# jluuser/PyTorch-VAE

Hardware: AMD Instinct MI355X
Metric: train images/sec @64x64x3 bs256 (curve tensors [B,64,6], SURVEY.md s0) (higher is better)
Workload: dtype f32; 1 GPU; C2: stage2_vq.yaml model with num_quantizers=1 K=512 D=64 N=64; full train step (fwd+loss+bwd+clip+AdamW+EMA), dropout 0.1, loss weights at epoch 100; per_gpu_batch=256, global_batch=256, seq_len=64, parallelism=dp1, hipgraph=True, params=43115078

## Files before the change

### pytorch-vae_amd/csrc/attention.hip

```cpp
#include "common.h"

namespace {

__device__ __forceinline__ int kmap(int r, int h) { return (r & 3) + 8 * (r >> 2) + 4 * h; }

__device__ __forceinline__ f32x4 ld4_guard(const float* p, bool ok) {
    f32x4 z = {0.f, 0.f, 0.f, 0.f};
    return ok ? *reinterpret_cast<const f32x4*>(p) : z;
}

struct AttnArgs {
    const float* Q; int ldq;
    const float* K; int ldk;
    const float* V; int ldv;
    float* O; int ldo;
    float* LSE;
    const unsigned char* kvalid;
    int B, nh, T, S;
    long long qbs, kbs, vbs;
    float scale;
    DropCfg drop;
    const float* dO; int lddo;
    float* Dsum;
    float* dQ; int lddq;
// ... 819 lines not shown
        hipError_t e = hipFuncSetAttribute(reinterpret_cast<const void*>(&attn_bwd_small4_kernel<DH>),
                                           hipFuncAttributeMaxDynamicSharedMemorySize, (int)smem);
        if (e != hipSuccess) {
            vqh_set_error(hipGetErrorString(e));
            return VQH_ERR_LAUNCH;
        }
        attr_set = true;
    }
    hipLaunchKernelGGL((attn_bwd_small4_kernel<DH>), dim3(1, a.nh, a.B), dim3(256), smem, stream, a);
    VQH_LAUNCH_CHECK();
    return VQH_OK;
}

template <int DH>
int launch_bwd_small(const AttnArgs& a, hipStream_t stream) {
    if (!(g_attn_flags & 2)) return launch_bwd_small4<DH>(a, stream);
    static bool attr_set = false;
    const size_t smem = (size_t)(4 * 64 * (DH + 4) + 3 * 64) * sizeof(float);
    if (!attr_set) {
        hipError_t e = hipFuncSetAttribute(reinterpret_cast<const void*>(&attn_bwd_small_kernel<DH>),
                                           hipFuncAttributeMaxDynamicSharedMemorySize, (int)smem);
        if (e != hipSuccess) {
            vqh_set_error(hipGetErrorString(e));
            return VQH_ERR_LAUNCH;
        }
        attr_set = true;
    }
    hipLaunchKernelGGL((attn_bwd_small_kernel<DH>), dim3(1, a.nh, a.B), dim3(256), smem, stream, a);
    VQH_LAUNCH_CHECK();
    return VQH_OK;
}

int g_attn_flags = 0;

}

extern "C" int vqh_attn_set_flags(int flags) { const int old = g_attn_flags; g_attn_flags = flags; return old; }

extern "C" int vqh_attn_fwd(const float* Q, int ldq, const float* K, int ldk, const float* V, int ldv, float* O,
                            int ldo, float* LSE, const unsigned char* kvalid, int B, int nh, int T, int S, int dh,
                            int qkv_shared, const unsigned long long* rng_state, unsigned drop_site, float drop_p,
                            hipStream_t stream) {
    VQH_CHECK_ARG(B >= 0 && nh > 0 && T >= 0 && S >= 0, "vqh_attn_fwd: bad shape");
    VQH_CHECK_ARG(dh == 16 || dh == 32 || dh == 64, "vqh_attn_fwd: head dim must be 16/32/64");
    if (B == 0 || T == 0) return VQH_OK;
    VQH_CHECK_ARG(S > 0, "vqh_attn_fwd: no keys");
    VQH_CHECK_ARG(Q && K && V && O, "vqh_attn_fwd: null pointer");
    VQH_CHECK_ARG(aligned16(Q, ldq) && aligned16(K, ldk) && aligned16(V, ldv), "vqh_attn_fwd: operands must be 16-byte aligned");
    VQH_CHECK_ARG(drop_p == 0.f || rng_state, "vqh_attn_fwd: dropout needs rng_state");
    AttnArgs a{};
    a.Q = Q; a.ldq = ldq; a.K = K; a.ldk = ldk; a.V = V; a.ldv = ldv; a.O = O; a.ldo = ldo; a.LSE = LSE;
    a.kvalid = kvalid; a.B = B; a.nh = nh; a.T = T; a.S = S; a.scale = 1.0f / sqrtf((float)dh);
    a.qbs = (qkv_shared & 1) ? 0 : (long long)T * ldq; a.kbs = (qkv_shared & 2) ? 0 : (long long)S * ldk; a.vbs = (qkv_shared & 2) ? 0 : (long long)S * ldv;
    a.drop = make_drop(rng_state, drop_site, drop_p);
    if (T <= 64 && S <= 64 && aligned16(O, ldo) && !(g_attn_flags & 1)) {
        dim3 grid(1, nh, B);
        if (dh == 64 && !(g_attn_flags & (2 | 4))) {
            static bool attr_set = false;
            const int smem = 2 * ax::IMG + 2 * 128 * 4;
            if (!attr_set) {
                hipError_t e = hipFuncSetAttribute(reinterpret_cast<const void*>(&attn_fwd_small_x3_kernel),
                                                   hipFuncAttributeMaxDynamicSharedMemorySize, smem);
                if (e != hipSuccess) { vqh_set_error(hipGetErrorString(e)); return VQH_ERR_LAUNCH; }
                attr_set = true;
            }
            hipLaunchKernelGGL(attn_fwd_small_x3_kernel, grid, dim3(256), smem, stream, a);
            VQH_LAUNCH_CHECK();
            return VQH_OK;
        }
        if (!(g_attn_flags & 2)) {
            switch (dh) {
                case 16: hipLaunchKernelGGL((attn_fwd_small4_kernel<16>), grid, dim3(256), 0, stream, a); break;
                case 32: hipLaunchKernelGGL((attn_fwd_small4_kernel<32>), grid, dim3(256), 0, stream, a); break;
                default: hipLaunchKernelGGL((attn_fwd_small4_kernel<64>), grid, dim3(256), 0, stream, a); break;
            }
            VQH_LAUNCH_CHECK();
            return VQH_OK;
        }
        switch (dh) {
            case 16: hipLaunchKernelGGL((attn_fwd_small_kernel<16>), grid, dim3(128), 0, stream, a); break;
            case 32: hipLaunchKernelGGL((attn_fwd_small_kernel<32>), grid, dim3(128), 0, stream, a); break;
            default: hipLaunchKernelGGL((attn_fwd_small_kernel<64>), grid, dim3(128), 0, stream, a); break;
        }
        VQH_LAUNCH_CHECK();
        return VQH_OK;
    }
    const int NWq = (T >= 128) ? 4 : 2;
    dim3 grid((T + 32 * NWq - 1) / (32 * NWq), nh, B);
    if (dh == 64 && !(g_attn_flags & 4) && aligned16(O, ldo)) {
        static bool attr_x3[2] = {false, false};
        const void* fn = (NWq == 4) ? reinterpret_cast<const void*>(&attn_fwd_x3_kernel<4>) : reinterpret_cast<const void*>(&attn_fwd_x3_kernel<2>);
        if (!attr_x3[NWq == 4]) {
            hipError_t e = hipFuncSetAttribute(fn, hipFuncAttributeMaxDynamicSharedMemorySize, 2 * ax::IMG);
            if (e != hipSuccess) { vqh_set_error(hipGetErrorString(e)); return VQH_ERR_LAUNCH; }
            attr_x3[NWq == 4] = true;
        }
        if (NWq == 4) hipLaunchKernelGGL((attn_fwd_x3_kernel<4>), grid, dim3(256), 2 * ax::IMG, stream, a);
// ... 15 lines not shown
}

extern "C" int vqh_attn_bwd(const float* Q, int ldq, const float* K, int ldk, const float* V, int ldv,
                            const float* O, int ldo, const float* LSE, const float* dO, int lddo, float* Dsum,
                            float* dQ, int lddq, float* dK, int lddk, float* dV, int lddv,
                            const unsigned char* kvalid, int B, int nh, int T, int S, int dh, int qkv_shared,
                            const unsigned long long* rng_state, unsigned drop_site, float drop_p,
                            hipStream_t stream) {
    VQH_CHECK_ARG(B >= 0 && nh > 0 && T >= 0 && S >= 0, "vqh_attn_bwd: bad shape");
    VQH_CHECK_ARG(dh == 16 || dh == 32 || dh == 64, "vqh_attn_bwd: head dim must be 16/32/64");
    if (B == 0 || T == 0 || S == 0) return VQH_OK;
    VQH_CHECK_ARG(Q && K && V && O && LSE && dO && Dsum && dQ && dK && dV, "vqh_attn_bwd: null pointer");
    VQH_CHECK_ARG(aligned16(Q, ldq) && aligned16(K, ldk) && aligned16(V, ldv) && aligned16(O, ldo) && aligned16(dO, lddo),
                  "vqh_attn_bwd: operands must be 16-byte aligned");
    VQH_CHECK_ARG(drop_p == 0.f || rng_state, "vqh_attn_bwd: dropout needs rng_state");
    AttnArgs a{};
    a.Q = Q; a.ldq = ldq; a.K = K; a.ldk = ldk; a.V = V; a.ldv = ldv; a.O = const_cast<float*>(O); a.ldo = ldo;
    a.LSE = const_cast<float*>(LSE); a.kvalid = kvalid; a.B = B; a.nh = nh; a.T = T; a.S = S;
    a.scale = 1.0f / sqrtf((float)dh);
    a.qbs = (qkv_shared & 1) ? 0 : (long long)T * ldq; a.kbs = (qkv_shared & 2) ? 0 : (long long)S * ldk; a.vbs = (qkv_shared & 2) ? 0 : (long long)S * ldv;
    a.drop = make_drop(rng_state, drop_site, drop_p);
    a.dO = dO; a.lddo = lddo; a.Dsum = Dsum; a.dQ = dQ; a.lddq = lddq; a.dK = dK; a.lddk = lddk; a.dV = dV; a.lddv = lddv;
    if (T <= 64 && S <= 64 && aligned16(dQ, lddq) && aligned16(dK, lddk) && aligned16(dV, lddv) && !(g_attn_flags & 1)) {
        int rc = VQH_OK;
        if (dh == 64 && !(g_attn_flags & (2 | 4))) {
            static bool attr_set = false;
            const int smem = 2 * 64 * (ax::DH + 4) * 4 + 64 * (ax::DH + 4) * 4;
            if (!attr_set) {
                hipError_t e = hipFuncSetAttribute(reinterpret_cast<const void*>(&attn_bwd_small_x3_kernel),
                                                   hipFuncAttributeMaxDynamicSharedMemorySize, smem);
                if (e != hipSuccess) { vqh_set_error(hipGetErrorString(e)); return VQH_ERR_LAUNCH; }
                attr_set = true;
            }
            hipLaunchKernelGGL(attn_bwd_small_x3_kernel, dim3(1, nh, B), dim3(256), smem, stream, a);
            VQH_LAUNCH_CHECK();
            return VQH_OK;
        }
        switch (dh) {
            case 16: rc = launch_bwd_small<16>(a, stream); break;
            case 32: rc = launch_bwd_small<32>(a, stream); break;
            default: rc = launch_bwd_small<64>(a, stream); break;
        }
        return rc;
    }
    const int NWq = (T >= 128) ? 4 : 2, NWk = (S >= 128) ? 4 : 2;
    dim3 gq((T + 32 * NWq - 1) / (32 * NWq), nh, B), gk((S + 32 * NWk - 1) / (32 * NWk), nh, B);
    if (dh == 64 && !(g_attn_flags & 4) && aligned16(dQ, lddq) && aligned16(dK, lddk) && aligned16(dV, lddv)) {
        static bool attr_b[4] = {false, false, false, false};
        const int smem_q = 2 * ax::IMG, smem_k = 2 * ax::IMG + 3 * 64 * 4;
        const void* fq = (NWq == 4) ? reinterpret_cast<const void*>(&attn_bwd_dq_x3_kernel<4>) : reinterpret_cast<const void*>(&attn_bwd_dq_x3_kernel<2>);
        const void* fk = (NWk == 4) ? reinterpret_cast<const void*>(&attn_bwd_dkv_x3_kernel<4>) : reinterpret_cast<const void*>(&attn_bwd_dkv_x3_kernel<2>);
        if (!attr_b[NWq == 4]) {
            hipError_t e = hipFuncSetAttribute(fq, hipFuncAttributeMaxDynamicSharedMemorySize, smem_q);
            if (e != hipSuccess) { vqh_set_error(hipGetErrorString(e)); return VQH_ERR_LAUNCH; }
            attr_b[NWq == 4] = true;
        }
        if (!attr_b[2 + (NWk == 4)]) {
            hipError_t e = hipFuncSetAttribute(fk, hipFuncAttributeMaxDynamicSharedMemorySize, smem_k);
            if (e != hipSuccess) { vqh_set_error(hipGetErrorString(e)); return VQH_ERR_LAUNCH; }
            attr_b[2 + (NWk == 4)] = true;
        }
        if (NWq == 4) hipLaunchKernelGGL((attn_bwd_dq_x3_kernel<4>), gq, dim3(256), smem_q, stream, a);
        else hipLaunchKernelGGL((attn_bwd_dq_x3_kernel<2>), gq, dim3(128), smem_q, stream, a);
        if (NWk == 4) hipLaunchKernelGGL((attn_bwd_dkv_x3_kernel<4>), gk, dim3(256), smem_k, stream, a);
        else hipLaunchKernelGGL((attn_bwd_dkv_x3_kernel<2>), gk, dim3(128), smem_k, stream, a);
        VQH_LAUNCH_CHECK();
// ... 19 lines not shown
```

### pytorch-vae_amd/csrc/attention_x3.inc

```
typedef unsigned ax_u32x2 __attribute__((ext_vector_type(2)));
typedef unsigned ax_u32x4 __attribute__((ext_vector_type(4)));
typedef short ax_s16x4 __attribute__((ext_vector_type(4)));
typedef __bf16 ax_bf16x8 __attribute__((ext_vector_type(8)));
typedef __bf16 ax_bf16x2 __attribute__((ext_vector_type(2)));
typedef float ax_f32x2 __attribute__((ext_vector_type(2)));

__device__ __forceinline__ void ax_split2(float a0, float a1, unsigned& h, unsigned& m, unsigned& l) {
    h = __builtin_bit_cast(unsigned, __builtin_convertvector(ax_f32x2{a0, a1}, ax_bf16x2));
    const float r0 = a0 - __uint_as_float(h << 16), r1 = a1 - __uint_as_float(h & 0xffff0000u);
    m = __builtin_bit_cast(unsigned, __builtin_convertvector(ax_f32x2{r0, r1}, ax_bf16x2));
    const float s0 = r0 - __uint_as_float(m << 16), s1 = r1 - __uint_as_float(m & 0xffff0000u);
    l = __builtin_bit_cast(unsigned, __builtin_convertvector(ax_f32x2{s0, s1}, ax_bf16x2));
}

namespace ax {
constexpr int DH = 64, CK = 64;
constexpr int PLANE = CK * DH * 2;
constexpr int IMG = 3 * PLANE;
__device__ __forceinline__ int off(int row, int c) { return row * 128 + ((c ^ ((((row >> 1) & 1) << 2) | ((row >> 2) & 3))) << 4); }
}

template <int NT>
struct AxChunk {
    static constexpr int N = 1024 / NT;
    f32x4 v[N];
    __device__ __forceinline__ void load(const float* __restrict__ src, int ld, int row0, int nrows, int tid) {
#pragma unroll
        for (int j = 0; j < N; ++j) {
            const int i = tid + j * NT, r = row0 + (i >> 4), c = (i & 15) * 4;
            const int rr = max(min(r, nrows - 1), 0);
            v[j] = *reinterpret_cast<const f32x4*>(src + (size_t)rr * ld + c);
        }
#pragma unroll
        for (int j = 0; j < N; ++j) {
            const int i = tid + j * NT, r = row0 + (i >> 4);
            if (r >= nrows) v[j] = f32x4{0.f, 0.f, 0.f, 0.f};
        }
    }
    __device__ __forceinline__ void store(unsigned char* __restrict__ img, int tid, float scale = 1.f) const {
#pragma unroll
        for (int j = 0; j < N; ++j) {
            const int i = tid + j * NT, r = i >> 4, c4 = i & 15;
            unsigned h0, m0, l0, h1, m1, l1;
            ax_split2(v[j][0] * scale, v[j][1] * scale, h0, m0, l0);
            ax_split2(v[j][2] * scale, v[j][3] * scale, h1, m1, l1);
            const int o = ax::off(r, c4 >> 1) + (c4 & 1) * 8;
            *reinterpret_cast<ax_u32x2*>(img + o) = ax_u32x2{h0, h1};
            *reinterpret_cast<ax_u32x2*>(img + ax::PLANE + o) = ax_u32x2{m0, m1};
            *reinterpret_cast<ax_u32x2*>(img + 2 * ax::PLANE + o) = ax_u32x2{l0, l1};
        }
    }
};

__device__ __forceinline__ f32x16 ax_mma6(const ax_u32x4 (&a)[3], const ax_u32x4 (&b)[3], f32x16 acc) {
    acc = __builtin_amdgcn_mfma_f32_32x32x16_bf16(__builtin_bit_cast(ax_bf16x8, a[2]), __builtin_bit_cast(ax_bf16x8, b[0]), acc, 0, 0, 0);
    acc = __builtin_amdgcn_mfma_f32_32x32x16_bf16(__builtin_bit_cast(ax_bf16x8, a[0]), __builtin_bit_cast(ax_bf16x8, b[2]), acc, 0, 0, 0);
    acc = __builtin_amdgcn_mfma_f32_32x32x16_bf16(__builtin_bit_cast(ax_bf16x8, a[1]), __builtin_bit_cast(ax_bf16x8, b[1]), acc, 0, 0, 0);
    acc = __builtin_amdgcn_mfma_f32_32x32x16_bf16(__builtin_bit_cast(ax_bf16x8, a[1]), __builtin_bit_cast(ax_bf16x8, b[0]), acc, 0, 0, 0);
    acc = __builtin_amdgcn_mfma_f32_32x32x16_bf16(__builtin_bit_cast(ax_bf16x8, a[0]), __builtin_bit_cast(ax_bf16x8, b[1]), acc, 0, 0, 0);
    acc = __builtin_amdgcn_mfma_f32_32x32x16_bf16(__builtin_bit_cast(ax_bf16x8, a[0]), __builtin_bit_cast(ax_bf16x8, b[0]), acc, 0, 0, 0);
    return acc;
}

__device__ __forceinline__ void ax_split8(const float* p, ax_u32x4 (&out)[3]) {
    unsigned h[4], m[4], l[4];
#pragma unroll
    for (int i = 0; i < 4; ++i) ax_split2(p[2 * i], p[2 * i + 1], h[i], m[i], l[i]);
    out[0] = ax_u32x4{h[0], h[1], h[2], h[3]};
    out[1] = ax_u32x4{m[0], m[1], m[2], m[3]};
    out[2] = ax_u32x4{l[0], l[1], l[2], l[3]};
// ... 673 lines not shown
    if (h == 0) Sx[kh * 64 + q] = lsum;
    __syncthreads();
    const float ltot = Sx[q] + Sx[64 + q];
    const float inv = 1.f / ltot;
    float* Os = reinterpret_cast<float*>(Kimg);
#pragma unroll
    for (int pass = 0; pass < 2; ++pass) {
        if (kh == pass && q0 < a.T) {
#pragma unroll
            for (int d = 0; d < 2; ++d)
#pragma unroll
                for (int g4 = 0; g4 < 4; ++g4) {
                    f32x4 x;
#pragma unroll
                    for (int e = 0; e < 4; ++e) x[e] = o[d][4 * g4 + e];
                    float* dst = Os + q * LDO + d * 32 + 8 * g4 + 4 * h;
                    if (pass == 1) {
                        x += *reinterpret_cast<const f32x4*>(dst);
                        x *= inv;
                    }
                    *reinterpret_cast<f32x4*>(dst) = x;
                }
        }
        __syncthreads();
    }
    if (kh == 0 && h == 0 && a.LSE && q < a.T) a.LSE[rowbase + q] = m + __logf(ltot);
    float* Ob = a.O + (size_t)b * a.T * a.ldo + hh * DH;
#pragma unroll
    for (int i = tid; i < 64 * 16; i += 256) {
        const int r = i >> 4, c = (i & 15) * 4;
        if (r < a.T) *reinterpret_cast<f32x4*>(Ob + (size_t)r * a.ldo + c) = *reinterpret_cast<const f32x4*>(Os + r * LDO + c);
    }
}
```

### pytorch-vae_amd/csrc/rowwise.hip

```cpp
#include "common.h"
#include <stdlib.h>

namespace {

constexpr int WAVES_PER_BLOCK = 4;

__global__ __launch_bounds__(256) void layernorm_fwd_kernel(const float* __restrict__ x, int ldx,
                                                            const float* __restrict__ w, const float* __restrict__ b,
                                                            float* __restrict__ y, int ldy, float* __restrict__ mean,
                                                            float* __restrict__ rstd, int rows, int H, float eps) {
    const int lane = threadIdx.x & 63;
    const int row = blockIdx.x * WAVES_PER_BLOCK + (threadIdx.x >> 6);
    if (row >= rows) return;
    const float* xr = x + (size_t)row * ldx;
    float s = 0.f;
    for (int i = lane; i < H; i += 64) s += xr[i];
    const float mu = wave_sum(s) / (float)H;
    float v = 0.f;
    for (int i = lane; i < H; i += 64) {
        const float d = xr[i] - mu;
        v += d * d;
    }
    const float rs = rsqrtf(wave_sum(v) / (float)H + eps);
    float* yr = y + (size_t)row * ldy;
// ... 277 lines not shown

__global__ __launch_bounds__(256) void colsum_kernel(const float* __restrict__ X, int ld, int M, int N,
                                                     float* __restrict__ part, int rows_per_block) {
    __shared__ float red[4][64];
    const int c = blockIdx.x * 64 + (threadIdx.x & 63);
    const int ry = threadIdx.x >> 6;
    const int r0 = blockIdx.y * rows_per_block;
    const int r1 = min(M, r0 + rows_per_block);
    float s = 0.f;
    if (c < N)
        for (int r = r0 + ry; r < r1; r += 4) s += X[(size_t)r * ld + c];
    red[ry][threadIdx.x & 63] = s;
    __syncthreads();
    if (ry == 0 && c < N)
        part[(size_t)blockIdx.y * N + c] = red[0][threadIdx.x] + red[1][threadIdx.x] + red[2][threadIdx.x] + red[3][threadIdx.x];
}

__global__ __launch_bounds__(256) void embed_fwd_kernel(const float* __restrict__ x, int ldx, int c0,
                                                        const float* __restrict__ W, const float* __restrict__ b,
                                                        const float* __restrict__ pe, float* __restrict__ out,
                                                        int rows, int L, int H, DropCfg drop) {
    unsigned dkey = 0;
    if (drop.p > 0.f) dkey = drop_key(drop, drop.rng_state[0], drop.rng_state[1]);
    const long long total = (long long)rows * H;
    for (long long e = (long long)blockIdx.x * blockDim.x + threadIdx.x; e < total; e += (long long)gridDim.x * blockDim.x) {
        const int r = (int)(e / H), hcol = (int)(e % H);
        const float* xr = x + (size_t)r * ldx + c0;
        float v = b[hcol] + W[hcol * 3 + 0] * xr[0] + W[hcol * 3 + 1] * xr[1] + W[hcol * 3 + 2] * xr[2];
        if (drop.p > 0.f) v *= drop_keep(drop, dkey, (unsigned long long)e);
        out[e] = v + pe[(size_t)(r % L) * H + hcol];
    }
}

__global__ __launch_bounds__(256) void embed_bwd_kernel(const float* __restrict__ dy, const float* __restrict__ x,
                                                        int ldx, int c0, float* __restrict__ part, int rows, int H,
                                                        int rows_per_block, DropCfg drop) {
    __shared__ float red[4][4][64];
    unsigned dkey = 0;
    if (drop.p > 0.f) dkey = drop_key(drop, drop.rng_state[0], drop.rng_state[1]);
    const int hcol = blockIdx.x * 64 + (threadIdx.x & 63);
    const int ry = threadIdx.x >> 6;
    const int r0 = blockIdx.y * rows_per_block, r1 = min(rows, r0 + rows_per_block);
    float a0 = 0.f, a1 = 0.f, a2 = 0.f, a3 = 0.f;
    if (hcol < H)
        for (int r = r0 + ry; r < r1; r += 4) {
            float d = dy[(size_t)r * H + hcol];
            if (drop.p > 0.f) d *= drop_keep(drop, dkey, (unsigned long long)r * H + hcol);
            const float* xr = x + (size_t)r * ldx + c0;
            a0 += d * xr[0];
            a1 += d * xr[1];
            a2 += d * xr[2];
            a3 += d;
        }
    const int l = threadIdx.x & 63;
    red[ry][0][l] = a0; red[ry][1][l] = a1; red[ry][2][l] = a2; red[ry][3][l] = a3;
    __syncthreads();
    if (ry == 0 && hcol < H) {
#pragma unroll
        for (int c = 0; c < 4; ++c)
            part[((size_t)blockIdx.y * 4 + c) * H + hcol] = red[0][c][l] + red[1][c][l] + red[2][c][l] + red[3][c][l];
    }
}

__global__ void bcast_rows_kernel(const float* __restrict__ p0, const float* __restrict__ p1, float* __restrict__ out,
                                  int B, long long n) {
    const long long total = (long long)B * n;
    for (long long e = (long long)blockIdx.x * blockDim.x + threadIdx.x; e < total; e += (long long)gridDim.x * blockDim.x) {
        const long long i = e % n;
        out[e] = p1 ? p0[i] + p1[i] : p0[i];
    }
}

__global__ void dropout_bwd_kernel(const float* __restrict__ dy, float* __restrict__ out, long long n, DropCfg drop) {
    const unsigned dkey = drop_key(drop, drop.rng_state[0], drop.rng_state[1]);
    const long long nq = (n + 3) / 4;
    for (long long q = (long long)blockIdx.x * blockDim.x + threadIdx.x; q < nq; q += (long long)gridDim.x * blockDim.x) {
        float f[4];
        drop4(drop, dkey, (unsigned long long)q, f);
#pragma unroll
        for (int e = 0; e < 4; ++e) {
            const long long i = q * 4 + e;
            if (i < n) out[i] = dy[i] * f[e];
        }
    }
}
// ... 91 lines not shown
                                                                   float* __restrict__ metrics, int i_loss, int i_reg) {
    __shared__ float red[4];
    float acc = 0.f;
    for (int k = threadIdx.x; k < K; k += 256) {
        const float pc = colsum[k] * invR;
        const float lg = logf(fmaxf(pc, 1e-12f));
        acc += pc * lg;
        g[k] = lambda * invR * (lg + (pc > 1e-12f ? 1.f : 0.f));
    }
    acc = wave_sum(acc);
    if ((threadIdx.x & 63) == 0) red[threadIdx.x >> 6] = acc;
    __syncthreads();
    if (threadIdx.x == 0) {
        const float reg = lambda * (red[0] + red[1] + red[2] + red[3]);
        metrics[i_loss] += reg;
        metrics[i_reg] = reg;
    }
}

__global__ void vq_mix_kernel(const float* __restrict__ ze, const float* __restrict__ zsoft, const float* __restrict__ zhard,
                              float alpha, float* __restrict__ out, long long n) {
    for (long long i = (long long)blockIdx.x * blockDim.x + threadIdx.x; i < n; i += (long long)gridDim.x * blockDim.x) {
        const float mix = __fadd_rn(__fmul_rn(1.f - alpha, zsoft[i]), __fmul_rn(alpha, zhard[i]));
        out[i] = __fadd_rn(ze[i], __fsub_rn(mix, ze[i]));
    }
}

inline int blocks_for(long long n, int per_block = 256, int cap = 4096) {
    long long b = (n + per_block - 1) / per_block;
    if (b < 1) b = 1;
    if (b > cap) b = cap;
    return (int)b;
}

}

extern "C" int vqh_layernorm_fwd(const float* x, int ldx, const float* w, const float* b, float* y, int ldy,
                                 float* mean, float* rstd, int rows, int H, float eps, hipStream_t stream) {
    VQH_CHECK_ARG(rows >= 0 && H > 0 && ldx >= H && ldy >= H, "vqh_layernorm_fwd: bad shape");
    if (rows == 0) return VQH_OK;
    VQH_CHECK_ARG(x && w && b && y, "vqh_layernorm_fwd: null pointer");
    const int grid = (rows + WAVES_PER_BLOCK - 1) / WAVES_PER_BLOCK;
    const bool vec = (H % 4 == 0) && H <= 1024 && ((ldx | ldy) % 4 == 0) &&
                     (((reinterpret_cast<uintptr_t>(x) | reinterpret_cast<uintptr_t>(y) | reinterpret_cast<uintptr_t>(w) |
                        reinterpret_cast<uintptr_t>(b)) & 15) == 0);
    if (vec) {
        const int gv = grid > 2048 ? 2048 : grid;
        if (H <= 256) hipLaunchKernelGGL((layernorm_fwd_vec_kernel<1>), dim3(gv), dim3(256), 0, stream, x, ldx, w, b, y, ldy, mean, rstd, rows, H, eps);
        else if (H <= 512) hipLaunchKernelGGL((layernorm_fwd_vec_kernel<2>), dim3(gv), dim3(256), 0, stream, x, ldx, w, b, y, ldy, mean, rstd, rows, H, eps);
        else hipLaunchKernelGGL((layernorm_fwd_vec_kernel<4>), dim3(gv), dim3(256), 0, stream, x, ldx, w, b, y, ldy, mean, rstd, rows, H, eps);
    } else {
        hipLaunchKernelGGL(layernorm_fwd_kernel, dim3(grid), dim3(256), 0, stream, x, ldx, w, b, y, ldy, mean, rstd, rows, H, eps);
    }
    VQH_LAUNCH_CHECK();
    return VQH_OK;
}

extern "C" int vqh_reduce_slabs(const float* slabs, int S, long long stride, long long n, float* out, float beta,
                                hipStream_t stream) {
    VQH_CHECK_ARG(S >= 0 && n >= 0, "vqh_reduce_slabs: bad shape");
    if (n == 0) return VQH_OK;
    hipLaunchKernelGGL(reduce_slabs_kernel, dim3((unsigned)((n + 63) / 64)), dim3(1024), 0, stream, slabs, S, stride, n, out, beta);
    VQH_LAUNCH_CHECK();
    return VQH_OK;
}

// ... 67 lines not shown
        hipLaunchKernelGGL(colsum_kernel, dim3((N + 63) / 64, rb), dim3(256), 0, stream, X, ld, M, N, workspace, rows_per_block);
    hipLaunchKernelGGL(reduce_slabs_kernel, dim3((N + 63) / 64), dim3(1024), 0, stream, workspace, rb, (long long)N,
                       (long long)N, out, beta);
    VQH_LAUNCH_CHECK();
    return VQH_OK;
}

extern "C" int vqh_embed_fwd(const float* x, int ldx, int col0, const float* W, const float* b, const float* pe,
                             float* out, int rows, int L, int H, const unsigned long long* rng_state,
                             unsigned drop_site, float drop_p, hipStream_t stream) {
    VQH_CHECK_ARG(rows >= 0 && L > 0 && H > 0 && ldx >= col0 + 3, "vqh_embed_fwd: bad shape");
    if (rows == 0) return VQH_OK;
    VQH_CHECK_ARG(x && W && b && pe && out, "vqh_embed_fwd: null pointer");
    VQH_CHECK_ARG(drop_p == 0.f || rng_state, "vqh_embed_fwd: dropout needs rng_state");
    DropCfg d = make_drop(rng_state, drop_site, drop_p);
    hipLaunchKernelGGL(embed_fwd_kernel, dim3(blocks_for((long long)rows * H)), dim3(256), 0, stream, x, ldx, col0, W, b,
                       pe, out, rows, L, H, d);
    VQH_LAUNCH_CHECK();
    return VQH_OK;
}

extern "C" int vqh_embed_bwd(const float* dy, const float* x, int ldx, int col0, float* dW, float* db, float beta,
                             int rows, int H, const unsigned long long* rng_state, unsigned drop_site, float drop_p,
                             float* workspace, long long workspace_floats, hipStream_t stream) {
    VQH_CHECK_ARG(rows >= 0 && H > 0, "vqh_embed_bwd: bad shape");
    VQH_CHECK_ARG(dy && x && dW && db && workspace, "vqh_embed_bwd: null pointer");
    VQH_CHECK_ARG(drop_p == 0.f || rng_state, "vqh_embed_bwd: dropout needs rng_state");
    int rb = (rows + 255) / 256;
    if (rb < 1) rb = 1;
    if (rb > 128) rb = 128;
    const int rpb = (rows + rb - 1) / rb > 0 ? (rows + rb - 1) / rb : 1;
    VQH_CHECK_ARG((long long)rb * 4 * H <= workspace_floats, "vqh_embed_bwd: workspace too small");
    DropCfg d = make_drop(rng_state, drop_site, drop_p);
    hipLaunchKernelGGL(embed_bwd_kernel, dim3((H + 63) / 64, rb), dim3(256), 0, stream, dy, x, ldx, col0, workspace, rows,
                       H, rpb, d);
    VQH_LAUNCH_CHECK();
    float* scratch = workspace + (size_t)rb * 4 * H;
    VQH_CHECK_ARG((long long)rb * 4 * H + 4 * H <= workspace_floats, "vqh_embed_bwd: workspace too small");
    hipLaunchKernelGGL(reduce_slabs_kernel, dim3((4 * H + 63) / 64), dim3(1024), 0, stream, workspace, rb,
                       (long long)4 * H, (long long)4 * H, scratch, 0.f);
    hipLaunchKernelGGL(embed_scatter_kernel, dim3((H + 255) / 256), dim3(256), 0, stream, scratch, dW, db, beta, H);
    VQH_LAUNCH_CHECK();
    return VQH_OK;
}

extern "C" int vqh_bcast_rows(const float* p0, const float* p1, float* out, int B, long long n, hipStream_t stream) {
    VQH_CHECK_ARG(B >= 0 && n >= 0, "vqh_bcast_rows: bad shape");
    if (B == 0 || n == 0) return VQH_OK;
    hipLaunchKernelGGL(bcast_rows_kernel, dim3(blocks_for((long long)B * n)), dim3(256), 0, stream, p0, p1, out, B, n);
    VQH_LAUNCH_CHECK();
    return VQH_OK;
}

extern "C" int vqh_dropout_bwd(const float* dy, float* out, long long n, const unsigned long long* rng_state,
                               unsigned drop_site, float drop_p, hipStream_t stream) {
    VQH_CHECK_ARG(n >= 0 && drop_p > 0.f && drop_p < 1.f && rng_state, "vqh_dropout_bwd: bad argument");
    if (n == 0) return VQH_OK;
    DropCfg d = make_drop(rng_state, drop_site, drop_p);
    hipLaunchKernelGGL(dropout_bwd_kernel, dim3(blocks_for((n + 3) / 4)), dim3(256), 0, stream, dy, out, n, d);
    VQH_LAUNCH_CHECK();
    return VQH_OK;
}

extern "C" int vqh_add(const float* a, const float* b, float* out, long long n, hipStream_t stream) {
    VQH_CHECK_ARG(n >= 0, "vqh_add: bad n");
    if (n == 0) return VQH_OK;
    hipLaunchKernelGGL(add_kernel, dim3(blocks_for(n)), dim3(256), 0, stream, a, b, out, n);
    VQH_LAUNCH_CHECK();
// ... 71 lines not shown
```

Baseline: 9636 images/s.

## Add persistent pipelined small-attention kernels and vectorized embedding backward

Adds persistent-grid forward and backward attention kernels for small sequences that loop over (batch, head) items and issue global loads for the next item before writing out the current one. This is meant to hide load latency behind compute and output stores. These kernels are gated behind attention flag bit 8, which is off by default. The change also adds a float4-vectorized embedding backward kernel, used by default when alignment allows, with contraction control to keep the arithmetic matching the scalar kernel.

Result: no change. 9634 images/s (-0.0%).

```diff
diff --git a/pytorch-vae_amd/csrc/attention.hip b/pytorch-vae_amd/csrc/attention.hip
--- a/pytorch-vae_amd/csrc/attention.hip
+++ b/pytorch-vae_amd/csrc/attention.hip
@@ -875,6 +875,19 @@
 }
 
 int g_attn_flags = 0;
+
+int pipe_grid(int items) {
+    static int cus[64] = {0};
+    int dev = 0;
+    if (hipGetDevice(&dev) != hipSuccess || dev < 0 || dev >= 64) dev = 0;
+    if (cus[dev] == 0) {
+        int n = 0;
+        if (hipDeviceGetAttribute(&n, hipDeviceAttributeMultiprocessorCount, dev) != hipSuccess || n <= 0) n = 256;
+        cus[dev] = n;
+    }
+    const int g = 3 * cus[dev];
+    return items < g ? items : g;
+}
 
 }
 
@@ -906,6 +919,19 @@
                                                    hipFuncAttributeMaxDynamicSharedMemorySize, smem);
                 if (e != hipSuccess) { vqh_set_error(hipGetErrorString(e)); return VQH_ERR_LAUNCH; }
                 attr_set = true;
+            }
+            if (g_attn_flags & 8) {
+                static bool attr_pipe = false;
+                if (!attr_pipe) {
+                    hipError_t e = hipFuncSetAttribute(reinterpret_cast<const void*>(&attn_fwd_small_x3_pipe_kernel),
+                                                       hipFuncAttributeMaxDynamicSharedMemorySize, smem);
+                    if (e != hipSuccess) { vqh_set_error(hipGetErrorString(e)); return VQH_ERR_LAUNCH; }
+                    attr_pipe = true;
+                }
+                const int items = B * nh;
+                hipLaunchKernelGGL(attn_fwd_small_x3_pipe_kernel, dim3(pipe_grid(items)), dim3(256), smem, stream, a, items);
+                VQH_LAUNCH_CHECK();
+                return VQH_OK;
             }
             hipLaunchKernelGGL(attn_fwd_small_x3_kernel, grid, dim3(256), smem, stream, a);
             VQH_LAUNCH_CHECK();
@@ -987,6 +1013,19 @@
                 if (e != hipSuccess) { vqh_set_error(hipGetErrorString(e)); return VQH_ERR_LAUNCH; }
                 attr_set = true;
             }
+            if (g_attn_flags & 8) {
+                static bool attr_pipe = false;
+                if (!attr_pipe) {
+                    hipError_t e = hipFuncSetAttribute(reinterpret_cast<const void*>(&attn_bwd_small_x3_pipe_kernel),
+                                                       hipFuncAttributeMaxDynamicSharedMemorySize, smem);
+                    if (e != hipSuccess) { vqh_set_error(hipGetErrorString(e)); return VQH_ERR_LAUNCH; }
+                    attr_pipe = true;
+                }
+                const int items = B * nh;
+                hipLaunchKernelGGL(attn_bwd_small_x3_pipe_kernel, dim3(pipe_grid(items)), dim3(256), smem, stream, a, items);
+                VQH_LAUNCH_CHECK();
+                return VQH_OK;
+            }
             hipLaunchKernelGGL(attn_bwd_small_x3_kernel, dim3(1, nh, B), dim3(256), smem, stream, a);
             VQH_LAUNCH_CHECK();
             return VQH_OK;
diff --git a/pytorch-vae_amd/csrc/attention_x3.inc b/pytorch-vae_amd/csrc/attention_x3.inc
--- a/pytorch-vae_amd/csrc/attention_x3.inc
+++ b/pytorch-vae_amd/csrc/attention_x3.inc
@@ -24,18 +24,24 @@
 struct AxChunk {
     static constexpr int N = 1024 / NT;
     f32x4 v[N];
-    __device__ __forceinline__ void load(const float* __restrict__ src, int ld, int row0, int nrows, int tid) {
+    __device__ __forceinline__ void issue(const float* __restrict__ src, int ld, int row0, int nrows, int tid) {
 #pragma unroll
         for (int j = 0; j < N; ++j) {
             const int i = tid + j * NT, r = row0 + (i >> 4), c = (i & 15) * 4;
             const int rr = max(min(r, nrows - 1), 0);
             v[j] = *reinterpret_cast<const f32x4*>(src + (size_t)rr * ld + c);
         }
+    }
+    __device__ __forceinline__ void fill(int row0, int nrows, int tid) {
 #pragma unroll
         for (int j = 0; j < N; ++j) {
             const int i = tid + j * NT, r = row0 + (i >> 4);
             if (r >= nrows) v[j] = f32x4{0.f, 0.f, 0.f, 0.f};
         }
+    }
+    __device__ __forceinline__ void load(const float* __restrict__ src, int ld, int row0, int nrows, int tid) {
+        issue(src, ld, row0, nrows, tid);
+        fill(row0, nrows, tid);
     }
     __device__ __forceinline__ void store(unsigned char* __restrict__ img, int tid, float scale = 1.f) const {
 #pragma unroll
@@ -775,3 +781,412 @@
         if (r < a.T) *reinterpret_cast<f32x4*>(Ob + (size_t)r * a.ldo + c) = *reinterpret_cast<const f32x4*>(Os + r * LDO + c);
     }
 }
+
+
+__device__ __forceinline__ int ax_opaque(int x) {
+    asm volatile("" : "+v"(x));
+    return x;
+}
+
+struct AxRow {
+    f32x4 v[8];
+    __device__ __forceinline__ void issue(const float* rowp, int h) {
+#pragma unroll
+        for (int s = 0; s < 4; ++s) {
+            v[2 * s] = *reinterpret_cast<const f32x4*>(rowp + 16 * s + 8 * h);
+            v[2 * s + 1] = *reinterpret_cast<const f32x4*>(rowp + 16 * s + 8 * h + 4);
+        }
+    }
+    __device__ __forceinline__ void planes(bool ok, float scale, ax_u32x4 (&f)[4][3]) const {
+        const f32x4 z = {0.f, 0.f, 0.f, 0.f};
+#pragma unroll
+        for (int s = 0; s < 4; ++s) {
+            f32x4 x0 = ok ? v[2 * s] : z, x1 = ok ? v[2 * s + 1] : z;
+            x0 *= scale; x1 *= scale;
+            const float t[8] = {x0[0], x0[1], x0[2], x0[3], x1[0], x1[1], x1[2], x1[3]};
+            ax_split8(t, f[s]);
+        }
+    }
+};
+
+__device__ __forceinline__ void ax_fwd_item_issue(const AttnArgs& a, int item, int q, int h, int tid, AxChunk<256>& ck,
+                                                  AxChunk<256>& cv, AxRow& qr) {
+    const int hh = item % a.nh, b = item / a.nh;
+    const float* Qb = a.Q + (size_t)b * a.qbs + hh * ax::DH;
+    ck.issue(a.K + (size_t)b * a.kbs + hh * ax::DH, a.ldk, 0, a.S, tid);
+    cv.issue(a.V + (size_t)b * a.vbs + hh * ax::DH, a.ldv, 0, a.S, tid);
+    qr.issue(Qb + (size_t)min(q, a.T - 1) * a.ldq, h);
+}
+
+__device__ __forceinline__ void ax_fwd_item_out(const AttnArgs& a, int item, int tid, const float* Os, bool lse_out, size_t row,
+                                                float lse) {
+    constexpr int LDO = ax::DH + 4;
+    const int hh = item % a.nh, b = item / a.nh;
+    if (lse_out) a.LSE[row] = lse;
+    float* Ob = a.O + (size_t)b * a.T * a.ldo + hh * ax::DH;
+#pragma unroll
+    for (int j = 0; j < 4; ++j) {
+        const int i = tid + j * 256, r = i >> 4, c = (i & 15) * 4;
+        if (r < a.T) *reinterpret_cast<f32x4*>(Ob + (size_t)r * a.ldo + c) = *reinterpret_cast<const f32x4*>(Os + r * LDO + c);
+    }
+}
+
+__global__ __launch_bounds__(256, 3) void attn_fwd_small_x3_pipe_kernel(const AttnArgs a, const int items) {
+    constexpr int DH = ax::DH, LDO = DH + 4;
+    extern __shared__ __attribute__((aligned(16))) unsigned char ax_smem[];
+    unsigned char* Kimg = ax_smem;
+    unsigned char* Vimg = ax_smem + ax::IMG;
+    float* Mx = reinterpret_cast<float*>(ax_smem + 2 * ax::IMG);
+    float* Sx = Mx + 128;
+    unsigned long long seed = 0, step = 0;
+    if (a.drop.p > 0.f) { seed = a.drop.rng_state[0]; step = a.drop.rng_state[1]; }
+    AxChunk<256> ck, cv;
+    AxRow qr;
+    int item = blockIdx.x;
+    {
+        const int tid = threadIdx.x, lane = tid & 63, wave = tid >> 6;
+        ax_fwd_item_issue(a, item, (wave & 1) * 32 + (lane & 31), lane >> 5, tid, ck, cv, qr);
+    }
+    for (;;) {
+        const int tid = ax_opaque(threadIdx.x);
+        const int lane = tid & 63, wave = tid >> 6, l31 = lane & 31, h = lane >> 5;
+        const int qh = wave & 1, kh = wave >> 1;
+        const int q0 = qh * 32, s0 = kh * 32;
+        const int q = q0 + l31;
+        const bool active = (q0 < a.T) && (s0 < a.S);
+        const int hh = item % a.nh, b = item / a.nh;
+        const unsigned char* kv = a.kvalid ? a.kvalid + (size_t)b * a.S : nullptr;
+        const size_t rowbase = ((size_t)b * a.nh + hh) * a.T;
+        ax_u32x4 qf[4][3];
+        __syncthreads();
+        ck.fill(0, a.S, tid);
+        cv.fill(0, a.S, tid);
+        qr.planes(q < a.T, a.scale, qf);
+        ck.store(Kimg, tid);
+        cv.store(Vimg, tid);
+        __syncthreads();
+        f32x16 o[2];
+#pragma unroll
+        for (int d = 0; d < 2; ++d)
+#pragma unroll
+            for (int r = 0; r < 16; ++r) o[d][r] = 0.f;
+        f32x16 sacc;
+#pragma unroll
+        for (int r = 0; r < 16; ++r) sacc[r] = 0.f;
+        unsigned int vmask = 0;
+        float mloc = -INFINITY;
+        if (active) {
+#pragma unroll
+            for (int s = 0; s < 4; ++s) {
+                ax_u32x4 kf[3];
+                ax_read_rows(Kimg, s0 + l31, s, h, kf);
+                sacc = ax_mma6(kf, qf[s], sacc);
+            }
+            const int keyl = s0 + l31;
+            const unsigned char vb = (kv && keyl < a.S) ? kv[keyl] : (unsigned char)1;
+            vmask = (unsigned int)__ballot((keyl < a.S) && vb != 0);
+#pragma unroll
+            for (int r = 0; r < 16; ++r) mloc = ((vmask >> kmap(r, h)) & 1u) ? fmaxf(mloc, sacc[r]) : mloc;
+            mloc = fmaxf(mloc, __shfl_xor(mloc, 32, 64));
+        }
+        if (h == 0) Mx[kh * 64 + q] = mloc;
+        __syncthreads();
+        const float m = fmaxf(Mx[q], Mx[64 + q]);
+        float lsum = 0.f;
+        if (active) {
+            float p[16];
+#pragma unroll
+            for (int r = 0; r < 16; ++r) {
+                p[r] = ((vmask >> kmap(r, h)) & 1u) ? __expf(sacc[r] - m) : 0.f;
+                lsum += p[r];
+            }
+            lsum += __shfl_xor(lsum, 32, 64);
+            if (a.drop.p > 0.f) {
+                const unsigned rowkey = attn_rowkey(a.drop, seed, step, (unsigned long long)(rowbase + q));
+#pragma unroll
+                for (int r = 0; r < 16; ++r) p[r] *= attn_keep(a.drop, rowkey, s0 + kmap(r, h));
+            }
+#pragma unroll
+            for (int s = 0; s < 2; ++s) {
+                ax_u32x4 pf[3];
+                ax_split8(p + 8 * s, pf);
+#pragma unroll
+                for (int blk = 0; blk < 2; ++blk) {
+                    ax_u32x4 vf[3];
+#pragma unroll
+                    for (int pl = 0; pl < 3; ++pl) vf[pl] = ax_read_tr(Vimg + pl * ax::PLANE, s0 + 16 * s, blk, lane);
+                    o[blk] = ax_mma6(vf, pf, o[blk]);
+                }
+            }
+        }
+        if (h == 0) Sx[kh * 64 + q] = lsum;
+        __syncthreads();
+        const float ltot = Sx[q] + Sx[64 + q];
+        const float inv = 1.f / ltot;
+        float* Os = reinterpret_cast<float*>(Kimg);
+#pragma unroll
+        for (int pass = 0; pass < 2; ++pass) {
+            if (kh == pass && q0 < a.T) {
+#pragma unroll
+                for (int d = 0; d < 2; ++d)
+#pragma unroll
+                    for (int g4 = 0; g4 < 4; ++g4) {
+                        f32x4 x;
+#pragma unroll
+                        for (int e = 0; e < 4; ++e) x[e] = o[d][4 * g4 + e];
+                        float* dst = Os + q * LDO + d * 32 + 8 * g4 + 4 * h;
+                        if (pass == 1) {
+                            x += *reinterpret_cast<const f32x4*>(dst);
+                            x *= inv;
+                        }
+                        *reinterpret_cast<f32x4*>(dst) = x;
+                    }
+            }
+            __syncthreads();
+        }
+        const float lse = m + __logf(ltot);
+        const bool lse_out = kh == 0 && h == 0 && a.LSE && q < a.T;
+        const int next = item + (int)gridDim.x;
+        if (next >= items) {
+            ax_fwd_item_out(a, item, ax_opaque(tid), Os, lse_out, rowbase + q, lse);
+            break;
+        }
+        ax_fwd_item_issue(a, next, q, h, ax_opaque(tid), ck, cv, qr);
+        ax_fwd_item_out(a, item, ax_opaque(tid), Os, lse_out, rowbase + q, lse);
+        item = next;
+    }
+}
+
+__device__ __forceinline__ void ax_bwd_item_issue(const AttnArgs& a, int item, int tid, AxChunk<256>& cq, AxChunk<256>& ck) {
+    const int hh = item % a.nh, b = item / a.nh;
+    cq.issue(a.Q + (size_t)b * a.qbs + hh * ax::DH, a.ldq, 0, a.T, tid);
+    ck.issue(a.K + (size_t)b * a.kbs + hh * ax::DH, a.ldk, 0, a.S, tid);
+}
+
+__device__ __forceinline__ void ax_bwd_item_out(const AttnArgs& a, int item, int tid, const float* dQs) {
+    constexpr int LDO = ax::DH + 4;
+    const float* dKs = dQs + 64 * LDO;
+    const float* dVs = dKs + 64 * LDO;
+    const int hh = item % a.nh, b = item / a.nh;
+    float* dQb = a.dQ + (size_t)b * a.T * a.lddq + hh * ax::DH;
+    float* dKb = a.dK + (size_t)b * a.S * a.lddk + hh * ax::DH;
+    float* dVb = a.dV + (size_t)b * a.S * a.lddv + hh * ax::DH;
+#pragma unroll
+    for (int j = 0; j < 4; ++j) {
+        const int i = tid + j * 256, r = i >> 4, c = (i & 15) * 4;
+        if (r < a.T) *reinterpret_cast<f32x4*>(dQb + (size_t)r * a.lddq + c) = *reinterpret_cast<const f32x4*>(dQs + r * LDO + c);
+        if (r < a.S) {
+            *reinterpret_cast<f32x4*>(dKb + (size_t)r * a.lddk + c) = *reinterpret_cast<const f32x4*>(dKs + r * LDO + c);
+            *reinterpret_cast<f32x4*>(dVb + (size_t)r * a.lddv + c) = *reinterpret_cast<const f32x4*>(dVs + r * LDO + c);
+        }
+    }
+}
+
+__global__ __launch_bounds__(256, 3) void attn_bwd_small_x3_pipe_kernel(const AttnArgs a, const int items) {
+    constexpr int DH = ax::DH, LDO = DH + 4;
+    extern __shared__ __attribute__((aligned(16))) unsigned char ax_smem[];
+    unsigned char* Qimg = ax_smem;
+    unsigned char* Oimg = ax_smem + ax::IMG;
+    unsigned char* Kimg = Oimg;
+    float* Ls = reinterpret_cast<float*>(ax_smem + 2 * ax::IMG);
+    float* Ds = Ls + 64;
+    unsigned* Rk = reinterpret_cast<unsigned*>(Ds + 64);
+    unsigned long long seed = 0, step = 0;
+    if (a.drop.p > 0.f) { seed = a.drop.rng_state[0]; step = a.drop.rng_state[1]; }
+    AxChunk<256> cq, ck;
+    int item = blockIdx.x;
+    ax_bwd_item_issue(a, item, threadIdx.x, cq, ck);
+    for (;;) {
+        const int tid = ax_opaque(threadIdx.x);
+        const int lane = tid & 63, wave = tid >> 6, l31 = lane & 31, h = lane >> 5;
+        const int qh = wave & 1, kh = wave >> 1;
+        const int q0 = qh * 32, s0 = kh * 32;
+        const int key = s0 + l31;
+        const bool kin = key < a.S;
+        const bool active = (q0 < a.T) && (s0 < a.S);
+        const int hh = item % a.nh, b = item / a.nh;
+        const float* Kb = a.K + (size_t)b * a.kbs + hh * DH;
+        const float* Vb = a.V + (size_t)b * a.vbs + hh * DH;
+        const unsigned char* kv = a.kvalid ? a.kvalid + (size_t)b * a.S : nullptr;
+        const size_t rowbase = ((size_t)b * a.nh + hh) * a.T;
+        const bool kok = kin && (!kv || kv[key]);
+
+        ax_u32x4 vf[4][3];
+        AxChunk<256> cdo, co;
+        AxRow vr;
+        __syncthreads();
+        cdo.issue(a.dO + (size_t)b * a.T * a.lddo + hh * DH, a.lddo, 0, a.T, ax_opaque(tid));
+        co.issue(a.O + (size_t)b * a.T * a.ldo + hh * DH, a.ldo, 0, a.T, ax_opaque(tid));
+        vr.issue(Vb + (size_t)min(key, a.S - 1) * a.ldv, h);
+        cq.fill(0, a.T, tid);
+        cq.store(Qimg, tid, a.scale);
+        ck.fill(0, a.S, tid);
+        ck.store(Kimg, tid);
+        if (tid < 64) {
+            Ls[tid] = (tid < a.T) ? a.LSE[rowbase + tid] : 0.f;
+            Rk[tid] = (a.drop.p > 0.f) ? attn_rowkey(a.drop, seed, step, (unsigned long long)(rowbase + tid)) : 0u;
+        }
+        __syncthreads();
+
+        f32x16 dk[2], dv[2];
+#pragma unroll
+        for (int d = 0; d < 2; ++d)
+#pragma unroll
+            for (int r = 0; r < 16; ++r) { dk[d][r] = 0.f; dv[d][r] = 0.f; }
+        ax_u32x4 dsf[2][3];
+#pragma unroll
+        for (int s = 0; s < 2; ++s)
+#pragma unroll
+            for (int pl = 0; pl < 3; ++pl) dsf[s][pl] = ax_u32x4{0u, 0u, 0u, 0u};
+        f32x16 sacc;
+#pragma unroll
+        for (int r = 0; r < 16; ++r) sacc[r] = 0.f;
+        if (active) {
+#pragma unroll
+            for (int s = 0; s < 4; ++s) {
+                ax_u32x4 qfr[3], kf[3];
+                ax_read_rows(Qimg, q0 + l31, s, h, qfr);
+                ax_read_rows(Kimg, key, s, h, kf);
+                sacc = ax_mma6(qfr, kf, sacc);
+            }
+        }
+        __syncthreads();
+        cdo.fill(0, a.T, tid);
+        co.fill(0, a.T, tid);
+        cdo.store(Oimg, tid);
+#pragma unroll
+        for (int j = 0; j < AxChunk<256>::N; ++j) {
+            const int i = tid + j * 256, r = i >> 4;
+            float dsum = cdo.v[j][0] * co.v[j][0] + cdo.v[j][1] * co.v[j][1] + cdo.v[j][2] * co.v[j][2] + cdo.v[j][3] * co.v[j][3];
+#pragma unroll
+            for (int off = 8; off >= 1; off >>= 1) dsum += __shfl_xor(dsum, off, 64);
+            if ((i & 15) == 0) Ds[r] = dsum;
+        }
+        vr.planes(kin, 1.f, vf);
+        __syncthreads();
+        if (active) {
+            float ds[16];
+            f32x16 dpacc;
+#pragma unroll
+            for (int r = 0; r < 16; ++r) dpacc[r] = 0.f;
+#pragma unroll
+            for (int s = 0; s < 4; ++s) {
+                ax_u32x4 ofr[3];
+                ax_read_rows(Oimg, q0 + l31, s, h, ofr);
+                dpacc = ax_mma6(ofr, vf[s], dpacc);
+            }
+            float pd[16];
+#pragma unroll
+            for (int r = 0; r < 16; ++r) {
+                const int ql = q0 + kmap(r, h);
+                const float keep = (a.drop.p > 0.f) ? attn_keep(a.drop, Rk[ql], key) : 1.f;
+                const bool ok = kok && (ql < a.T);
+                const float pe = __expf(fminf(sacc[r] - Ls[ql], 80.f));
+                const float p = ok ? pe : 0.f;
+                pd[r] = p * keep;
+                ds[r] = p * (dpacc[r] * keep - Ds[ql]);
+            }
+#pragma unroll
+            for (int s = 0; s < 2; ++s) {
+                ax_u32x4 pdf[3];
+                ax_split8(pd + 8 * s, pdf);
+                ax_split8(ds + 8 * s, dsf[s]);
+#pragma unroll
+                for (int blk = 0; blk < 2; ++blk) {
+                    ax_u32x4 ot[3], qt[3];
+#pragma unroll
+                    for (int pl = 0; pl < 3; ++pl) {
+                        ot[pl] = ax_read_tr(Oimg + pl * ax::PLANE, q0 + 16 * s, blk, lane);
+                        qt[pl] = ax_read_tr(Qimg + pl * ax::PLANE, q0 + 16 * s, blk, lane);
+                    }
+                    dv[blk] = ax_mma6(ot, pdf, dv[blk]);
+                    dk[blk] = ax_mma6(qt, dsf[s], dk[blk]);
+                }
+            }
+        }
+        __syncthreads();
+        {
+            AxChunk<256> ck2;
+            const int tid2 = ax_opaque(tid);
+            ck2.load(Kb, a.ldk, 0, a.S, tid2);
+            ck2.store(Kimg, tid2);
+            unsigned char* Simg = Qimg;
+#pragma unroll
+            for (int s = 0; s < 2; ++s)
+#pragma unroll
+                for (int pl = 0; pl < 3; ++pl)
+#pragma unroll
+                    for (int g2 = 0; g2 < 2; ++g2) {
+                        const int col = q0 + 8 * (2 * s + g2) + 4 * h;
+                        *reinterpret_cast<ax_u32x2*>(Simg + pl * ax::PLANE + ax::off(key, col >> 3) + (col & 7) * 2) =
+                            ax_u32x2{dsf[s][pl][2 * g2], dsf[s][pl][2 * g2 + 1]};
+                    }
+        }
+        __syncthreads();
+
+        const int blk2 = wave >> 1;
+        f32x16 dq;
+#pragma unroll
+        for (int r = 0; r < 16; ++r) dq[r] = 0.f;
+        const bool active2 = q0 < a.T;
+        if (active2) {
+#pragma unroll
+            for (int s = 0; s < 4; ++s) {
+                if (16 * s >= a.S) break;
+                ax_u32x4 kt[3], st[3];
+#pragma unroll
+                for (int pl = 0; pl < 3; ++pl) {
+                    kt[pl] = ax_read_tr(Kimg + pl * ax::PLANE, 16 * s, blk2, lane);
+                    st[pl] = ax_read_tr(Qimg + pl * ax::PLANE, 16 * s, qh, lane);
+                }
+                dq = ax_mma6(kt, st, dq);
+            }
+        }
+        __syncthreads();
+
+        float* dQs = reinterpret_cast<float*>(ax_smem);
+        float* dKs = dQs + 64 * LDO;
+        float* dVs = dKs + 64 * LDO;
+        {
+            float* dst = dQs + (q0 + l31) * LDO + blk2 * 32;
+#pragma unroll
+            for (int g4 = 0; g4 < 4; ++g4) {
+                f32x4 x;
+#pragma unroll
+                for (int e = 0; e < 4; ++e) x[e] = dq[4 * g4 + e] * a.scale;
+                *reinterpret_cast<f32x4*>(dst + 8 * g4 + 4 * h) = x;
+            }
+        }
+#pragma unroll
+        for (int pass = 0; pass < 2; ++pass) {
+            if (qh == pass) {
+                float* dst0 = dKs + key * LDO;
+                float* dst1 = dVs + key * LDO;
+#pragma unroll
+                for (int d = 0; d < 2; ++d)
+#pragma unroll
+                    for (int g4 = 0; g4 < 4; ++g4) {
+                        const int dd = d * 32 + 8 * g4 + 4 * h;
+                        f32x4 x0, x1;
+#pragma unroll
+                        for (int e = 0; e < 4; ++e) { x0[e] = dk[d][4 * g4 + e]; x1[e] = dv[d][4 * g4 + e]; }
+                        if (pass == 1) {
+                            x0 += *reinterpret_cast<const f32x4*>(dst0 + dd);
+                            x1 += *reinterpret_cast<const f32x4*>(dst1 + dd);
+                        }
+                        *reinterpret_cast<f32x4*>(dst0 + dd) = x0;
+                        *reinterpret_cast<f32x4*>(dst1 + dd) = x1;
+                    }
+            }
+            __syncthreads();
+        }
+        const int next = item + (int)gridDim.x;
+        if (next >= items) {
+            ax_bwd_item_out(a, item, ax_opaque(tid), dQs);
+            break;
+        }
+        ax_bwd_item_issue(a, next, ax_opaque(tid), cq, ck);
+        ax_bwd_item_out(a, item, ax_opaque(tid), dQs);
+        item = next;
+    }
+}
diff --git a/pytorch-vae_amd/csrc/rowwise.hip b/pytorch-vae_amd/csrc/rowwise.hip
--- a/pytorch-vae_amd/csrc/rowwise.hip
+++ b/pytorch-vae_amd/csrc/rowwise.hip
@@ -333,6 +333,75 @@
     }
 }
 
+__device__ __forceinline__ float embed_mul(float a, float b) {
+#pragma clang fp contract(off)
+    return a * b;
+}
+__device__ __forceinline__ void embed_bwd_acc(float d, float x0, float x1, float x2, float& a0, float& a1, float& a2, float& a3) {
+#pragma clang fp contract(off)
+    const float t = d * x0;
+    a0 = a0 + t;
+    a1 = __builtin_fmaf(d, x1, a1);
+    a2 = __builtin_fmaf(d, x2, a2);
+    a3 = a3 + d;
+}
+
+__global__ __launch_bounds__(256) void embed_bwd_vec_kernel(const float* __restrict__ dy, const float* __restrict__ x,
+                                                            int ldx, int c0, float* __restrict__ part, int rows, int H,
+                                                            int rows_per_block, DropCfg drop) {
+    __shared__ f32x4 red[4][4][64];
+    unsigned dkey = 0;
+    if (drop.p > 0.f) dkey = drop_key(drop, drop.rng_state[0], drop.rng_state[1]);
+    const int H4 = H >> 2;
+    const int l = threadIdx.x & 63, ry = threadIdx.x >> 6;
+    const int cq = blockIdx.x * 64 + l, hcol = cq * 4;
+    const int r0 = blockIdx.y * rows_per_block, r1 = min(rows, r0 + rows_per_block);
+    float a0[4] = {0.f, 0.f, 0.f, 0.f}, a1[4] = {0.f, 0.f, 0.f, 0.f}, a2[4] = {0.f, 0.f, 0.f, 0.f}, a3[4] = {0.f, 0.f, 0.f, 0.f};
+    if (cq < H4) {
+        int r = r0 + ry;
+        for (; r + 28 < r1; r += 32) {
+            f32x4 d[8];
+#pragma unroll
+            for (int u = 0; u < 8; ++u) d[u] = *reinterpret_cast<const f32x4*>(dy + (size_t)(r + 4 * u) * H + hcol);
+#pragma unroll
+            for (int u = 0; u < 8; ++u) {
+                const int ru = r + 4 * u;
+                if (drop.p > 0.f) {
+                    float f[4];
+                    drop4(drop, dkey, (unsigned long long)ru * H4 + cq, f);
+#pragma unroll
+                    for (int e = 0; e < 4; ++e) d[u][e] = embed_mul(d[u][e], f[e]);
+                }
+                const float* xr = x + (size_t)ru * ldx + c0;
+                const float x0 = xr[0], x1 = xr[1], x2 = xr[2];
+#pragma unroll
+                for (int e = 0; e < 4; ++e) embed_bwd_acc(d[u][e], x0, x1, x2, a0[e], a1[e], a2[e], a3[e]);
+            }
+        }
+        for (; r < r1; r += 4) {
+            f32x4 d = *reinterpret_cast<const f32x4*>(dy + (size_t)r * H + hcol);
+            if (drop.p > 0.f) {
+                float f[4];
+                drop4(drop, dkey, (unsigned long long)r * H4 + cq, f);
+#pragma unroll
+                for (int e = 0; e < 4; ++e) d[e] = embed_mul(d[e], f[e]);
+            }
+            const float* xr = x + (size_t)r * ldx + c0;
+            const float x0 = xr[0], x1 = xr[1], x2 = xr[2];
+#pragma unroll
+            for (int e = 0; e < 4; ++e) embed_bwd_acc(d[e], x0, x1, x2, a0[e], a1[e], a2[e], a3[e]);
+        }
+    }
+    red[ry][0][l] = f32x4{a0[0], a0[1], a0[2], a0[3]}; red[ry][1][l] = f32x4{a1[0], a1[1], a1[2], a1[3]};
+    red[ry][2][l] = f32x4{a2[0], a2[1], a2[2], a2[3]}; red[ry][3][l] = f32x4{a3[0], a3[1], a3[2], a3[3]};
+    __syncthreads();
+    if (ry == 0 && cq < H4) {
+#pragma unroll
+        for (int c = 0; c < 4; ++c)
+            *reinterpret_cast<f32x4*>(part + ((size_t)blockIdx.y * 4 + c) * H + hcol) = red[0][c][l] + red[1][c][l] + red[2][c][l] + red[3][c][l];
+    }
+}
+
 __global__ __launch_bounds__(256) void embed_bwd_kernel(const float* __restrict__ dy, const float* __restrict__ x,
                                                         int ldx, int c0, float* __restrict__ part, int rows, int H,
                                                         int rows_per_block, DropCfg drop) {
@@ -346,12 +415,9 @@
     if (hcol < H)
         for (int r = r0 + ry; r < r1; r += 4) {
             float d = dy[(size_t)r * H + hcol];
-            if (drop.p > 0.f) d *= drop_keep(drop, dkey, (unsigned long long)r * H + hcol);
+            if (drop.p > 0.f) d = embed_mul(d, drop_keep(drop, dkey, (unsigned long long)r * H + hcol));
             const float* xr = x + (size_t)r * ldx + c0;
-            a0 += d * xr[0];
-            a1 += d * xr[1];
-            a2 += d * xr[2];
-            a3 += d;
+            embed_bwd_acc(d, xr[0], xr[1], xr[2], a0, a1, a2, a3);
         }
     const int l = threadIdx.x & 63;
     red[ry][0][l] = a0; red[ry][1][l] = a1; red[ry][2][l] = a2; red[ry][3][l] = a3;
@@ -509,6 +575,8 @@
     if (b > cap) b = cap;
     return (int)b;
 }
+
+inline bool aligned16p(const void* p) { return (reinterpret_cast<uintptr_t>(p) & 15) == 0; }
 
 }
 
@@ -642,8 +710,12 @@
     const int rpb = (rows + rb - 1) / rb > 0 ? (rows + rb - 1) / rb : 1;
     VQH_CHECK_ARG((long long)rb * 4 * H <= workspace_floats, "vqh_embed_bwd: workspace too small");
     DropCfg d = make_drop(rng_state, drop_site, drop_p);
-    hipLaunchKernelGGL(embed_bwd_kernel, dim3((H + 63) / 64, rb), dim3(256), 0, stream, dy, x, ldx, col0, workspace, rows,
-                       H, rpb, d);
+    if ((H & 3) == 0 && aligned16p(dy) && aligned16p(workspace))
+        hipLaunchKernelGGL(embed_bwd_vec_kernel, dim3((H / 4 + 63) / 64, rb), dim3(256), 0, stream, dy, x, ldx, col0, workspace,
+                           rows, H, rpb, d);
+    else
+        hipLaunchKernelGGL(embed_bwd_kernel, dim3((H + 63) / 64, rb), dim3(256), 0, stream, dy, x, ldx, col0, workspace, rows,
+                           H, rpb, d);
     VQH_LAUNCH_CHECK();
     float* scratch = workspace + (size_t)rb * 4 * H;
     VQH_CHECK_ARG((long long)rb * 4 * H + 4 * H <= workspace_floats, "vqh_embed_bwd: workspace too small");
```
